# pyprob/pyprob

Hardware: NVIDIA H100
Metric: ic_train_traces_per_sec (higher is better)
Workload: dtype f32

## Files before the change

pyprob_b200/csrc/net.cu:

```cuda
#include <vector>
#include <string.h>
#include <stdlib.h>
#include <stdint.h>

#include "common.cuh"
#include "gemm_simt.cuh"
#include "heads.cuh"
#include "tc_grouped.cuh"
#include "tc_lstm.cuh"
#include "tc_cluster.cuh"
#include "tc_persist.cuh"
#include "obs_mlp.cuh"

using gemm::Problem;

struct HImg {
  float* k_hi = nullptr; float* k_lo = nullptr; float* mn_hi = nullptr; float* mn_lo = nullptr;
  int64_t kb = 0;
};

struct WImg {
  int64_t k_hi = 0, k_lo = 0, mn_hi = 0, mn_lo = 0;
  int kb = 0;
};
// ... 1174 lines not shown
  const int C2 = 2 * (D.type_dim + D.addr_dim);
  const bool one_pass = S <= 4 && H4 <= 2048;
  int max_rows = 0;
  for (int s = 0; s < d.NS; ++s) max_rows = b->step_nrows_host[s] > max_rows ? b->step_nrows_host[s] : max_rows;
  if (one_pass) {
    int slab = (d.R + 2 * PPB_NUM_SMS - 1) / (2 * PPB_NUM_SMS);
    slab = slab < 4 ? 4 : (slab > kRedSlab ? kRedSlab : slab);
    const dim3 g((max_rows + slab - 1) / slab, d.NS);
    const float* wt = d.T > 1 ? w.w_smp_t : w.p_step;
    if (H4 <= 1024)
      k_dgates_reduce<4><<<g, 256, 0, st>>>(dgates, wt, w.smp_emb, b->values, b->step_prev_addr, b->step_row0, b->step_nrows,
                                            b->row_prev, net->d_addrs, H4, S, I, E, w.d_pstep, grad, D.w_ih_off, slab);
    else
      k_dgates_reduce<8><<<g, 256, 0, st>>>(dgates, wt, w.smp_emb, b->values, b->step_prev_addr, b->step_row0, b->step_nrows,
                                            b->row_prev, net->d_addrs, H4, S, I, E, w.d_pstep, grad, D.w_ih_off, slab);
    PPB_LAUNCH_CHECK();
  } else {
    dim3 g((H4 + 31) / 32, d.NS);
    k_step_colsum<<<g, 256, 0, st>>>(dgates, b->step_row0, b->step_nrows, H4, w.d_pstep);
    PPB_LAUNCH_CHECK();
  }
  {
    const int jbs = (C2 + 31) / 32;
    int zsplit = PPB_NUM_SMS / 2 / (jbs * d.NS);
    zsplit = zsplit < 1 ? 1 : (zsplit > 16 ? 16 : zsplit);
    const int nx = jbs * d.NS * zsplit;
    const int nw = (int)(((int64_t)H4 * C2 + H4 + 255) / 256);
    k_pstep_bwd<<<nx + nw, 256, 0, st>>>(w.d_pstep, arena + D.w_ih_off, w.emb_cat, net->d_addrs, net->d_type_off, b->step_addr,
                                         b->step_prev_addr, d.NS, H4, I, E + S, D.type_dim, D.addr_dim, zsplit, nx, grad,
                                         D.w_ih_off, D.b_ih_off, D.b_hh_off);
    PPB_LAUNCH_CHECK();
  }
  if (d.T > 1 && !one_pass) {
    const int slab = 64;
    k_smp_bwd_seg<<<dim3((max_rows + slab - 1) / slab, d.NS), 128, 0, st>>>(dgates, w.w_smp_t, w.smp_emb, b->values,
                                                                           b->step_prev_addr, b->step_row0, b->step_nrows,
                                                                           b->row_prev, net->d_addrs, H4, S, slab, grad);
    PPB_LAUNCH_CHECK();
    int rpb = 1024;
    dim3 g((H4 + 255) / 256, (d.R + rpb - 1) / rpb);
    k_wsmp_grad<<<g, 256, 0, st>>>(dgates, w.smp_emb, d.R, H4, S, I, E, grad + D.w_ih_off, rpb);
    PPB_LAUNCH_CHECK();
  }
  return PPB_OK;
}

}

#include "net_tc.inc"
#include "net_ff.inc"

namespace {

int simt_loss_forward(ppb_net* net, const float* arena, const ppb_batch* b, void* workspace, float* loss_out,
                      int32_t* status_out, float* row_lp_out, int want_grad, cudaStream_t st) {
  PPB_CHECK_ARG(b->row_align == 1, "the SIMT path needs a batch encoded with row_align = 1");
  const ppb_net_desc& D = net->desc;
  Dims d = dims_of(b);
  Ws w = carve(net, d, workspace);
  const int H = D.lstm_dim, H4 = 4 * H, E = D.obs_dim, S = D.sample_dim, I = net->I;

  Builder bl;
  obs_fp32_plan_fwd(bl, D, arena, b->obs, d.B, w, w.obs_emb);
  const int ph_p = (int)bl.phases.size();
  bl.begin();
  bl.add(linear_fwd(w.obs_emb, E, arena + D.w_ih_off, I, nullptr, w.p_obs, H4, d.B, H4, E, 0));
  const int ph_rec0 = (int)bl.phases.size();
  for (int t = 1; t < d.T; ++t) {
    bl.begin();
    int r0 = b->row_off_host[t], n = b->row_off_host[t + 1] - r0, rp = b->row_off_host[t - 1];
    bl.add(linear_fwd(w.h + (int64_t)rp * H, H, arena + D.w_hh_off, H, nullptr, w.gates + (int64_t)r0 * H4, H4, n, H4, H, 0));
  }
  int ph_h1, ph_h2;
  simt_head_fwd(bl, net, arena, b, w, H, ph_h1, ph_h2);
  int rc = upload_and_get(net, bl, w.problems, w.max_problems / 2, st, 0);
  if (rc) return rc;

  PPB_CUDA(cudaMemsetAsync(w.loss_acc, 0, 256, st));
  for (int l = 0; l < ph_p; ++l) { rc = run_phase(bl.phases[l], w.problems, st); if (rc) return rc; }
  rc = launch_step_inputs_fwd(net, arena, b, w, st); if (rc) return rc;
  rc = run_phase(bl.phases[ph_p], w.problems, st, &bl); if (rc) return rc;
  for (int t = 0; t < d.T; ++t) {
    int r0 = b->row_off_host[t], n = b->row_off_host[t + 1] - r0;
    if (t > 0) { rc = run_phase(bl.phases[ph_rec0 + t - 1], w.problems, st, &bl); if (rc) return rc; }
    k_cell_fwd<<<ew_grid((int64_t)n * H), 256, 0, st>>>(w.gates, w.p_obs, w.p_step, w.w_smp_t, w.smp_emb, b->row_step,
                                                       b->row_prev, b->row_trace, w.c, w.h, HImg(), r0, n, H, S, t);
    PPB_LAUNCH_CHECK();
  }
  return simt_head_nll(net, b, w, bl, ph_h1, ph_h2, loss_out, status_out, row_lp_out, want_grad, st);
}

int simt_loss_backward(ppb_net* net, const float* arena, float* grad, const ppb_batch* b, void* workspace, float grad_scale,
                       cudaStream_t st) {
  PPB_CHECK_ARG(b->step_nrows_host, "missing per-step host arrays");
  const ppb_net_desc& D = net->desc;
  Dims d = dims_of(b);
  Ws w = carve(net, d, workspace);
  float* dgates = dgates_ptr(w, workspace);
  const int H = D.lstm_dim, H4 = 4 * H, E = D.obs_dim, I = net->I;

  PPB_CUDA(cudaMemsetAsync(w.d_pstep, 0, (size_t)d.NS * H4 * sizeof(float), st));
  if (grad_scale != 1.0f) {
    k_scale<<<ew_grid((int64_t)d.R * net->out_pad), 256, 0, st>>>(w.d_out, (int64_t)d.R * net->out_pad, grad_scale);
    PPB_LAUNCH_CHECK();
  }

  Builder bl;
  const int ph_dhid = 0, ph_hw = 1;
  simt_head_bwd(bl, net, arena, grad, b, w, H);
  const int ph_rec0 = 2;
  for (int t = d.T - 1; t >= 1; --t) {
    bl.begin();
    int r0 = b->row_off_host[t], n = b->row_off_host[t + 1] - r0;
    bl.add(linear_dx(dgates + (int64_t)r0 * H4, H4, arena + D.w_hh_off, H, w.dh_rec + (int64_t)b->row_off_host[t - 1] * H, H, n, H4, H, 0));
  }
  const int ph_lstm_w = (int)bl.phases.size();
  bl.begin();
  {
    int r1 = b->row_off_host[1 < d.T ? 1 : d.T];
    int n1 = d.R - r1;
    if (n1 > 0) {
      Problem p = linear_dw(dgates + (int64_t)r1 * H4, H4, w.h, H, grad + D.w_hh_off, H, n1, H4, H);
      p.kb_gather = b->row_prev + r1;
      bl.add(p);
    }
    bl.add(linear_dw(w.d_pobs, H4, w.obs_emb, E, grad + D.w_ih_off, I, d.B, H4, E));
    bl.add(linear_dx(w.d_pobs, H4, arena + D.w_ih_off, I, w.d_obs_emb, E, d.B, H4, E, 0));
  }
  const int ph_obs = obs_fp32_plan_bwd(bl, D, arena, grad, b->obs, d.B, w);
  Problem* dprobs = w.problems + w.max_problems / 2;
  int rc = upload_and_get(net, bl, dprobs, w.max_problems / 2, st, 1);
  if (rc) return rc;

  rc = run_phase(bl.phases[ph_dhid], dprobs, st); if (rc) return rc;
  rc = run_phase(bl.phases[ph_hw], dprobs, st); if (rc) return rc;
  rc = launch_head_bias_grad(net, b, w, grad, st); if (rc) return rc;
  for (int t = d.T - 1; t >= 0; --t) {
    int r0 = b->row_off_host[t], n = b->row_off_host[t + 1] - r0;
    int n_next = (t + 1 < d.T) ? b->row_off_host[t + 2] - b->row_off_host[t + 1] : 0;
    if (n_next > 0) { rc = run_phase(bl.phases[ph_rec0 + (d.T - 2 - t)], dprobs, st, &bl); if (rc) return rc; }
    k_cell_bwd<false><<<ew_grid((int64_t)n * H), 256, 0, st>>>(w.gates, w.c, w.dh, w.dh_rec, w.dc, dgates, w.d_pobs, b->row_prev,
                                                       b->row_next, b->row_trace, HImg(), r0, n, H, t, HImg());
    PPB_LAUNCH_CHECK();
  }
  rc = launch_step_inputs_bwd(net, arena, grad, b, w, dgates, st); if (rc) return rc;
  rc = run_phase(bl.phases[ph_lstm_w], dprobs, st, &bl); if (rc) return rc;
  return obs_fp32_bwd(bl, ph_obs, dprobs, D, grad, d.B, w, st);
}

}

extern "C" {

int ppb_net_create(ppb_net** out, const ppb_net_desc* d) {
  PPB_CHECK_ARG(out && d, "null argument");
  PPB_CHECK_ARG(d->network_type == PPB_NET_LSTM || d->network_type == PPB_NET_FEEDFORWARD, "unknown network type");
  if (d->network_type == PPB_NET_FEEDFORWARD)
    PPB_CHECK_ARG(d->obs_dim > 0 && d->lstm_dim == 0 && d->sample_dim == 0 && d->addr_dim == 0 && d->type_dim == 0,
                  "bad dims (a feed-forward net has obs_dim > 0 and no LSTM, sample, address or type embedding)");
  else
    PPB_CHECK_ARG(d->lstm_dim > 0 && d->obs_dim > 0 && d->sample_dim > 0 && d->sample_dim <= 8, "bad dims");
  PPB_CHECK_ARG(d->num_obs > 0 && d->num_obs <= PPB_MAX_OBS, "bad observable count");
  PPB_CHECK_ARG(d->mixture_k > 0 && d->mixture_k <= heads::KMAX, "mixture components must be in [1,32]");
  ppb_net* n = new ppb_net();
  n->desc = *d;
  n->I = d->obs_dim + d->sample_dim + 2 * (d->type_dim + d->addr_dim);
  const char* fc = getenv("PPB_FUSED_CELL");
  n->fused_cell = !(fc && fc[0] == '0');
  const char* hg = getenv("PPB_HOST_STEP_GRAPH");
  n->host_graph = (hg && hg[0] == '0') ? 0 : 1;
  for (int i = 0; i < 16; ++i) PPB_CUDA(cudaEventCreateWithFlags(&n->fork_ev[i], cudaEventDisableTiming));
  for (int i = 0; i < 2; ++i) PPB_CUDA(cudaStreamCreateWithFlags(&n->side[i], cudaStreamNonBlocking));
  *out = n;
  return PPB_OK;
}

int ppb_net_set_tables(ppb_net* net, const ppb_addr_desc* addrs, int32_t n_addrs, const int64_t* type_off,
                       int32_t n_types, int64_t arena_floats) {
  const bool ff = net && net->desc.network_type == PPB_NET_FEEDFORWARD;
  PPB_CHECK_ARG(net && addrs && n_addrs > 0 && (ff ? n_types == 0 : (type_off && n_types > 0)), "bad arguments");
  net->addrs.assign(addrs, addrs + n_addrs);
  net->type_off.assign(type_off, type_off + n_types);
  net->arena_floats = arena_floats;
  int dh = 4, op = 4;
  for (auto& a : net->addrs) {
    PPB_CHECK_ARG(a.family >= 0 && a.family <= PPB_FAMILY_BERNOULLI, "unknown family");
    PPB_CHECK_ARG(a.family != PPB_FAMILY_CATEGORICAL || (a.num_categories > 0 && a.num_categories <= heads::CMAX),
                  "categorical head: 1..128 categories supported");
    PPB_CHECK_ARG(a.family != PPB_FAMILY_BERNOULLI || (a.head_out == 1 && a.smp_in == 1 && a.num_categories == 0),
                  "bernoulli head: head_out = 1, smp_in = 1, num_categories = 0");
    PPB_CHECK_ARG(ff || (a.type_id >= 0 && a.type_id < n_types), "type id out of range");
    if (a.head_hidden > dh) dh = a.head_hidden;
    if (a.head_out > op) op = a.head_out;
  }
  net->dh_pad = (int)align_up(dh, 4);
  net->out_pad = (int)align_up(op, 4);
  if (net->d_addrs) cudaFree(net->d_addrs);
  if (net->d_type_off) cudaFree(net->d_type_off);
  net->d_type_off = nullptr;
  PPB_CUDA(cudaMalloc((void**)&net->d_addrs, sizeof(ppb_addr_desc) * n_addrs));
  PPB_CUDA(cudaMemcpy(net->d_addrs, addrs, sizeof(ppb_addr_desc) * n_addrs, cudaMemcpyHostToDevice));
  if (n_types > 0) {
    PPB_CUDA(cudaMalloc((void**)&net->d_type_off, sizeof(int64_t) * n_types));
    PPB_CUDA(cudaMemcpy(net->d_type_off, type_off, sizeof(int64_t) * n_types, cudaMemcpyHostToDevice));
  }
  return build_weight_images(net);
}

int ppb_net_destroy(ppb_net* net) {
  if (!net) return PPB_OK;
  if (net->d_addrs) cudaFree(net->d_addrs);
  if (net->d_type_off) cudaFree(net->d_type_off);
  for (int i = 0; i < 2; ++i) {
    if (net->h_stage[i]) cudaFreeHost(net->h_stage[i]);
    if (net->ev_stage[i]) cudaEventDestroy(net->ev_stage[i]);
    if (net->h_blob[i]) cudaFreeHost(net->h_blob[i]);
    if (net->ev_blob[i]) cudaEventDestroy(net->ev_blob[i]);
  }
  for (int i = 0; i < 2; ++i) if (net->side[i]) cudaStreamDestroy(net->side[i]);
  for (int i = 0; i < 16; ++i) if (net->fork_ev[i]) cudaEventDestroy(net->fork_ev[i]);
  if (net->wimg) cudaFree(net->wimg);
  if (net->d_pack) cudaFree(net->d_pack);
  if (net->whh_il) cudaFree(net->whh_il);
  if (net->d_lstm_steps) cudaFree(net->d_lstm_steps);
  if (net->host_exec) cudaGraphExecDestroy(net->host_exec);
  if (net->host_stream) cudaStreamDestroy(net->host_stream);
  if (net->host_hyper_dev) cudaFree(net->host_hyper_dev);
  if (net->host_state_dev) cudaFree(net->host_state_dev);
  if (net->host_pin) cudaFreeHost(net->host_pin);
  delete net;
  return PPB_OK;
}

int64_t ppb_ic_workspace_bytes(const ppb_net* net, int32_t n_traces, int32_t n_rows, int32_t t_max, int32_t n_steps,
                               int32_t n_groups) {
  if (!net || n_traces <= 0 || n_rows <= 0) return -1;
  Dims d; d.B = n_traces; d.R = n_rows; d.T = t_max; d.NS = n_steps; d.G = n_groups;
  return simt_region_bytes(net, d) + carve_tc(net, d, nullptr).total_bytes + 1024;
}

int ppb_ic_loss_forward(ppb_net* net, const float* arena, const ppb_batch* b, void* workspace,
                        int64_t workspace_bytes, int precision, float* loss_out, int32_t* status_out,
                        float* row_lp_out, int want_grad, void* stream) {
  int rc = check_batch(net, b);
  if (rc) return rc;
  PPB_CHECK_ARG(arena && workspace, "null arena/workspace");
  PPB_CHECK_ARG(!net->addrs.empty(), "address tables not set");
  PPB_CHECK_ARG(precision >= 0 && precision <= 2, "unknown precision mode");
  Dims d = dims_of(b);
  PPB_CHECK_ARG(workspace_bytes >= ppb_ic_workspace_bytes(net, d.B, d.R, d.T, d.NS, d.G), "workspace too small");
  cudaStream_t st = (cudaStream_t)stream;
  if (net->desc.network_type == PPB_NET_FEEDFORWARD)
    return ff_loss_forward(net, arena, b, workspace, precision, loss_out, status_out, row_lp_out, want_grad, st);
  if (precision != PPB_PREC_FP32_SIMT)
    return tc_loss_forward(net, arena, b, workspace, precision, loss_out, status_out, row_lp_out, want_grad, st);
  return simt_loss_forward(net, arena, b, workspace, loss_out, status_out, row_lp_out, want_grad, st);
}

int ppb_ic_loss_backward(ppb_net* net, const float* arena, float* grad, const ppb_batch* b, void* workspace,
                         int64_t workspace_bytes, int precision, float grad_scale, void* stream) {
  int rc = check_batch(net, b);
  if (rc) return rc;
  PPB_CHECK_ARG(arena && grad && workspace, "null arena/grad/workspace");
  Dims d = dims_of(b);
  PPB_CHECK_ARG(workspace_bytes >= ppb_ic_workspace_bytes(net, d.B, d.R, d.T, d.NS, d.G), "workspace too small");
  cudaStream_t st = (cudaStream_t)stream;
  if (net->desc.network_type == PPB_NET_FEEDFORWARD)
    return ff_loss_backward(net, arena, grad, b, workspace, precision, grad_scale, st);
  if (precision != PPB_PREC_FP32_SIMT) return tc_loss_backward(net, arena, grad, b, workspace, precision, grad_scale, st);
  return simt_loss_backward(net, arena, grad, b, workspace, grad_scale, st);
}

}

namespace {

__global__ void __launch_bounds__(256) k_adam(float* __restrict__ p, const float* __restrict__ g,
                                               float* __restrict__ m, float* __restrict__ v, int64_t n, float lr,
                                               float b1, float b2, float eps, float wd, float bc1, float bc2_sqrt,
                                               float gscale) {
  ppb_pdl_trigger();
  ppb_pdl_wait();
  int64_t n4 = n >> 2;
  float step = lr / bc1;
  for (int64_t q = (int64_t)blockIdx.x * blockDim.x + threadIdx.x; q < n4; q += (int64_t)gridDim.x * blockDim.x) {
    float4 pp = reinterpret_cast<float4*>(p)[q], gg = reinterpret_cast<const float4*>(g)[q];
    float4 mm = reinterpret_cast<float4*>(m)[q], vv = reinterpret_cast<float4*>(v)[q];
    float pa[4] = {pp.x, pp.y, pp.z, pp.w}, ga[4] = {gg.x, gg.y, gg.z, gg.w};
    float ma[4] = {mm.x, mm.y, mm.z, mm.w}, va[4] = {vv.x, vv.y, vv.z, vv.w};
#pragma unroll
    for (int j = 0; j < 4; ++j) ppb_adam_update(pa[j], ga[j], ma[j], va[j], b1, b2, eps, wd, gscale, step, bc2_sqrt);
    reinterpret_cast<float4*>(p)[q] = make_float4(pa[0], pa[1], pa[2], pa[3]);
    reinterpret_cast<float4*>(m)[q] = make_float4(ma[0], ma[1], ma[2], ma[3]);
    reinterpret_cast<float4*>(v)[q] = make_float4(va[0], va[1], va[2], va[3]);
  }
  for (int64_t i = (n4 << 2) + (int64_t)blockIdx.x * blockDim.x + threadIdx.x; i < n;
       i += (int64_t)gridDim.x * blockDim.x) {
    float pi = p[i], mi = m[i], vi = v[i];
    ppb_adam_update(pi, g[i], mi, vi, b1, b2, eps, wd, gscale, step, bc2_sqrt);
    m[i] = mi; v[i] = vi; p[i] = pi;
  }
}

__global__ void __launch_bounds__(256) k_adam_dev(float* __restrict__ p, const float* __restrict__ g,
                                                   float* __restrict__ m, float* __restrict__ v, int64_t n, int vec,
                                                   const float* __restrict__ hyper, long long* __restrict__ step_ctr,
                                                   float* __restrict__ bc1_out, unsigned int* __restrict__ done_ctr) {
  ppb_pdl_trigger();
  ppb_pdl_wait();
  __shared__ float s_bc[2];
  __shared__ long long s_t;
  const int64_t n4 = vec ? (n >> 2) : 0;
  const int64_t stride = (int64_t)gridDim.x * blockDim.x;
  int64_t q = (int64_t)blockIdx.x * blockDim.x + threadIdx.x;
  const float4 z4 = make_float4(0.f, 0.f, 0.f, 0.f);
  float4 gg = z4, mm = z4, vv = z4;
  if (q < n4) {
    gg = reinterpret_cast<const float4*>(g)[q];
    mm = reinterpret_cast<float4*>(m)[q];
    vv = reinterpret_cast<float4*>(v)[q];
  }
  if (threadIdx.x == 0) {
    long long t = *step_ctr + 1;
    s_t = t;
    s_bc[0] = (float)(1.0 - pow((double)hyper[1], (double)t));
    s_bc[1] = (float)sqrt(1.0 - pow((double)hyper[2], (double)t));
  }
  __syncthreads();
  const float lr = hyper[0], b1 = hyper[1], b2 = hyper[2], eps = hyper[3], wd = hyper[4], gscale = hyper[5];
  const float step = lr / s_bc[0], bc2_sqrt = s_bc[1];
  while (q < n4) {
    const bool zero = wd == 0.0f && gg.x == 0.0f && gg.y == 0.0f && gg.z == 0.0f && gg.w == 0.0f && mm.x == 0.0f &&
                      mm.y == 0.0f && mm.z == 0.0f && mm.w == 0.0f && vv.x == 0.0f && vv.y == 0.0f && vv.z == 0.0f &&
                      vv.w == 0.0f;
    if (!zero) {
      float4 pp = reinterpret_cast<float4*>(p)[q];
      ppb_adam_update(pp.x, gg.x, mm.x, vv.x, b1, b2, eps, wd, gscale, step, bc2_sqrt);
      ppb_adam_update(pp.y, gg.y, mm.y, vv.y, b1, b2, eps, wd, gscale, step, bc2_sqrt);
      ppb_adam_update(pp.z, gg.z, mm.z, vv.z, b1, b2, eps, wd, gscale, step, bc2_sqrt);
      ppb_adam_update(pp.w, gg.w, mm.w, vv.w, b1, b2, eps, wd, gscale, step, bc2_sqrt);
      reinterpret_cast<float4*>(p)[q] = pp;
      reinterpret_cast<float4*>(m)[q] = mm;
      reinterpret_cast<float4*>(v)[q] = vv;
    }
    q += stride;
    if (q < n4) {
      gg = reinterpret_cast<const float4*>(g)[q];
      mm = reinterpret_cast<float4*>(m)[q];
      vv = reinterpret_cast<float4*>(v)[q];
    }
  }
  for (int64_t i = (n4 << 2) + (int64_t)blockIdx.x * blockDim.x + threadIdx.x; i < n;
       i += (int64_t)gridDim.x * blockDim.x) {
    float pi = p[i], mi = m[i], vi = v[i];
    ppb_adam_update(pi, g[i], mi, vi, b1, b2, eps, wd, gscale, step, bc2_sqrt);
    m[i] = mi; v[i] = vi; p[i] = pi;
  }
  __syncthreads();
  if (threadIdx.x == 0) {
    __threadfence();
    if (atomicAdd(done_ctr, 1u) == gridDim.x - 1) {
      *step_ctr = s_t;
      *bc1_out = s_bc[0];
      *done_ctr = 0u;
    }
  }
}

__global__ void __launch_bounds__(256) k_cell_infer(const float* __restrict__ rec, const float* __restrict__ p_row,
                                                     const float* __restrict__ w_smp_t,
                                                     const float* __restrict__ smp_emb, float* __restrict__ c,
                                                     float* __restrict__ h, int64_t n, int H, int S, int first) {
  int64_t total = n * H;
  for (int64_t e = (int64_t)blockIdx.x * blockDim.x + threadIdx.x; e < total; e += (int64_t)gridDim.x * blockDim.x) {
    int64_t i = e / H;
    int j = (int)(e % H);
    float pre[4];
#pragma unroll
    for (int g = 0; g < 4; ++g) {
      int col = g * H + j;
      float v = p_row[col];
      if (!first) {
        v += rec[i * 4 * H + col];
        for (int s = 0; s < S; ++s) v = fmaf(smp_emb[i * S + s], w_smp_t[(int64_t)s * 4 * H + col], v);
      }
      pre[g] = v;
    }
    float ig = ppb_cell_sigmoid(pre[0]);
    float fg = ppb_cell_sigmoid(pre[1]);
    float gg = ppb_cell_tanh(pre[2]);
    float og = ppb_cell_sigmoid(pre[3]);
    float cp = first ? 0.0f : c[i * H + j];
    float cn = fg * cp + ig * gg;
    c[i * H + j] = cn;
    h[i * H + j] = og * ppb_cell_tanh(cn);
  }
}

__global__ void k_smp_embed_infer(const float* __restrict__ arena, ppb_addr_desc a, const float* __restrict__ value,
                                  int64_t n, int S, float* __restrict__ smp_emb) {
  for (int64_t e = (int64_t)blockIdx.x * blockDim.x + threadIdx.x; e < n * S; e += (int64_t)gridDim.x * blockDim.x) {
    int64_t i = e / S;
    int j = (int)(e % S);
    smp_emb[e] = fmaxf(smp_embed_pre(arena, a, value[i], j), 0.0f);
  }
}

__global__ void k_step_row_infer(const float* __restrict__ arena, ppb_addr_desc prev, int has_prev, ppb_addr_desc cur,
                                 const int64_t* __restrict__ type_off, int td, int ad, float* __restrict__ row) {
  int C2 = 2 * (td + ad);
  for (int j = threadIdx.x; j < C2; j += blockDim.x) {
    const int64_t o = step_embed_off(type_off, td, ad, j, [&](bool is_prev, const ppb_addr_desc*& a) {
      a = is_prev ? &prev : &cur;
      return !is_prev || has_prev;
    });
    row[j] = o >= 0 ? arena[o] : 0.0f;
  }
}

__global__ void __launch_bounds__(128) k_head_params(const float* __restrict__ out_raw, int out_pad, ppb_addr_desc a,
                                                      int K, const float* __restrict__ prior0, int s0,
                                                      const float* __restrict__ prior1, int s1,
                                                      float* __restrict__ params, int64_t n) {
  for (int64_t i = (int64_t)blockIdx.x * blockDim.x + threadIdx.x; i < n; i += (int64_t)gridDim.x * blockDim.x) {
    const float* x = out_raw + i * out_pad;
    if (a.family == PPB_FAMILY_BERNOULLI) {
      params[i] = heads::bernoulli_prob(x[0]);
    } else if (a.family == PPB_FAMILY_CATEGORICAL) {
      float xs[heads::CMAX], q[heads::CMAX];
      for (int c = 0; c < a.num_categories; ++c) xs[c] = x[c];
      heads::categorical_probs(xs, a.num_categories, q);
      for (int c = 0; c < a.num_categories; ++c) params[i * a.num_categories + c] = q[c];
    } else {
      float xs[3 * heads::KMAX], mean[heads::KMAX], sd[heads::KMAX], pr[heads::KMAX], lo, hi;
      for (int j = 0; j < 3 * K; ++j) xs[j] = x[j];
      float p0 = prior0 ? prior0[i * s0] : 0.0f, p1 = prior1 ? prior1[i * s1] : 0.0f;
      heads::mixture_params(a.family, xs, K, p0, p1, mean, sd, pr, &lo, &hi);
      for (int k = 0; k < K; ++k) {
        params[i * 3 * K + k] = mean[k];
        params[i * 3 * K + K + k] = sd[k];
        params[i * 3 * K + 2 * K + k] = pr[k];
      }
    }
  }
}

struct InferWs {
  HImg h_img, hid_img;
  tcg::Problem* tprobs;
  float *gates, *hid, *out_raw, *smp_emb, *p_row, *emb_row, *w_smp_t;
  float* obs_act[PPB_MAX_OBS][PPB_MAX_FF_LAYERS];
  float* obs_cat;
  float* fin_act[PPB_MAX_FF_LAYERS];
  Problem* problems;
  int64_t max_problems, total_bytes;
};

InferWs carve_infer(const ppb_net* net, int64_t n, void* base) {
  const ppb_net_desc& D = net->desc;
  InferWs w;
  memset(&w, 0, sizeof(w));
  char* p = (char*)base;
  int64_t off = 0;
  auto take = [&](int64_t floats) { float* r = (float*)(p + off); off += align_up(floats * 4, 256); return r; };
  const int H4 = 4 * D.lstm_dim;
  w.gates = take(n * H4);
  w.hid = take(n * net->dh_pad);
  w.out_raw = take(n * net->out_pad);
  w.smp_emb = take(n * D.sample_dim);
  w.p_row = take(H4);
  w.emb_row = take(2 * (D.type_dim + D.addr_dim));
  w.w_smp_t = take((int64_t)D.sample_dim * H4);
  for (int j = 0; j < D.num_obs; ++j)
    for (int l = 0; l + 1 < D.obs_ff[j].num_layers; ++l) w.obs_act[j][l] = take(n * D.obs_ff[j].layers[l].out_dim);
  w.obs_cat = take(n * D.obs_dim);
  for (int l = 0; l + 1 < D.obs_final.num_layers; ++l) w.fin_act[l] = take(n * D.obs_final.layers[l].out_dim);
  w.max_problems = 64 + 2LL * PPB_MAX_OBS * PPB_MAX_FF_LAYERS;
  w.problems = (Problem*)take(w.max_problems * (int64_t)(sizeof(Problem) / 4));
  auto img_k = [&](int64_t rows, int64_t cols) {
    HImg im;
    int64_t nfl = img_floats(rows, cols);
    off = align_up(off, 1024);
    im.kb = (cols + 31) / 32;
    im.k_hi = take(nfl); im.k_lo = take(nfl);
    return im;
  };
  w.h_img = img_k(n, D.lstm_dim);
  w.hid_img = img_k(n, net->dh_pad);
  w.tprobs = (tcg::Problem*)take(8 * (int64_t)(sizeof(tcg::Problem) / 4));
  w.total_bytes = off;
  return w;
}

}

extern "C" {

int ppb_prof_enable(int on) {
  for (auto& sp : g_prof.spans) { cudaEventDestroy(sp.first); cudaEventDestroy(sp.second); }
  g_prof.spans.clear();
  g_prof.flops = 0.0;
  g_prof.launches = 0;
  g_prof.on = on != 0;
  return PPB_OK;
}

int ppb_prof_read(double* total_ms_out, int64_t* launches_out, double* flops_out) {
  double total = 0.0;
  for (auto& sp : g_prof.spans) {
    PPB_CUDA(cudaEventSynchronize(sp.second));
    float ms = 0.0f;
    PPB_CUDA(cudaEventElapsedTime(&ms, sp.first, sp.second));
    total += ms;
  }
  if (total_ms_out) *total_ms_out = total;
  if (launches_out) *launches_out = g_prof.launches;
  if (flops_out) *flops_out = g_prof.flops;
  return PPB_OK;
}

int64_t ppb_sizeof(int which) {
  switch (which) {
    case 0: return sizeof(ppb_net_desc);
    case 1: return sizeof(ppb_addr_desc);
    case 2: return sizeof(ppb_batch);
    case 3: return sizeof(ppb_ff_desc);
    case 4: return sizeof(ppb_linear_desc);
    default: return -1;
  }
}

int ppb_batch_from_image(const void* image_host, const void* image_dev, int64_t image_bytes, ppb_batch* out) {
  PPB_CHECK_ARG(image_host && out, "null image");
  const int64_t* hd = (const int64_t*)image_host;
  PPB_CHECK_ARG(image_bytes >= (int64_t)(PPB_IMAGE_HEADER_WORDS * 8), "image too small");
  PPB_CHECK_ARG(hd[0] == PPB_IMAGE_MAGIC, "bad batch image magic");
  PPB_CHECK_ARG(hd[8] == image_bytes, "image size mismatch");
  memset(out, 0, sizeof(*out));
  out->n_traces = (int32_t)hd[1]; out->n_sub = (int32_t)hd[2]; out->t_max = (int32_t)hd[3];
  out->n_rows = (int32_t)hd[4]; out->n_steps = (int32_t)hd[5]; out->n_groups = (int32_t)hd[6];
  out->obs_in_total = (int32_t)hd[7];
  for (int k = 9; k < 9 + 19; ++k)
    PPB_CHECK_ARG(hd[k] >= PPB_IMAGE_HEADER_WORDS * 8 && hd[k] < image_bytes && (hd[k] & 15) == 0, "bad array offset");
  out->row_align = (int32_t)hd[28];
  PPB_CHECK_ARG(out->row_align == 1 || out->row_align == 128, "row_align must be 1 or 128");
  const char* Hh = (const char*)image_host;
  const char* Dv = (const char*)image_dev;
  out->row_off_host = (const int32_t*)(Hh + hd[9]);
  out->group_addr_host = (const int32_t*)(Hh + hd[10]);
  out->group_start_host = (const int32_t*)(Hh + hd[11]);
  out->step_addr_host = (const int32_t*)(Hh + hd[13]);
  out->step_row0_host = (const int32_t*)(Hh + hd[15]);
  out->step_nrows_host = (const int32_t*)(Hh + hd[16]);
  out->step_t_host = (const int32_t*)(Hh + hd[26]);
  out->step_prev_row0_host = (const int32_t*)(Hh + hd[27]);
  if (Dv) {
    out->trace_sub = (const int32_t*)(Dv + hd[12]);
    out->step_addr = (const int32_t*)(Dv + hd[13]);
    out->step_prev_addr = (const int32_t*)(Dv + hd[14]);
    out->step_row0 = (const int32_t*)(Dv + hd[15]);
    out->step_nrows = (const int32_t*)(Dv + hd[16]);
    out->row_step = (const int32_t*)(Dv + hd[17]);
    out->row_prev = (const int32_t*)(Dv + hd[18]);
    out->values = (const float*)(Dv + hd[19]);
    out->prior0 = (const float*)(Dv + hd[20]);
    out->prior1 = (const float*)(Dv + hd[21]);
    out->obs = (const float*)(Dv + hd[22]);
    out->head_rows = (const int32_t*)(Dv + hd[23]);
    out->row_trace = (const int32_t*)(Dv + hd[24]);
    out->row_next = (const int32_t*)(Dv + hd[25]);
    out->step_t = (const int32_t*)(Dv + hd[26]);
    out->step_prev_row0 = (const int32_t*)(Dv + hd[27]);
    out->group_addr = (const int32_t*)(Dv + hd[10]);
    out->group_start = (const int32_t*)(Dv + hd[11]);
  }
  return PPB_OK;
}

int ppb_adam_step(float* arena, const float* grad, float* exp_avg, float* exp_avg_sq, int64_t n, float lr, float beta1,
                  float beta2, float eps, float weight_decay, int64_t step, float grad_scale, void* stream) {
  PPB_CHECK_ARG(arena && grad && exp_avg && exp_avg_sq && n > 0 && step >= 1, "bad arguments");
  double bc1 = 1.0 - pow((double)beta1, (double)step), bc2 = 1.0 - pow((double)beta2, (double)step);
  PPB_CUDA(ppb_launch(k_adam, dim3(ppb_grid_for(n, 256, 4)), dim3(256), 0, (cudaStream_t)stream, 0, 0, arena, grad, exp_avg,
                      exp_avg_sq, n, lr, beta1, beta2, eps, weight_decay, (float)bc1, (float)sqrt(bc2), grad_scale));
  PPB_LAUNCH_CHECK();
  return PPB_OK;
}

int ppb_adam_step_dev(float* arena, const float* grad, float* exp_avg, float* exp_avg_sq, int64_t n,
                      const float* hyper_dev, void* state_dev, void* stream) {
  PPB_CHECK_ARG(arena && grad && exp_avg && exp_avg_sq && hyper_dev && state_dev && n > 0, "bad arguments");
  const int vec = ((((uintptr_t)arena | (uintptr_t)grad | (uintptr_t)exp_avg | (uintptr_t)exp_avg_sq) & 15) == 0) ? 1 : 0;
  PPB_CUDA(ppb_launch(k_adam_dev, dim3(ppb_grid_for(n, 256, 4)), dim3(256), 0, (cudaStream_t)stream, 0, 0, arena, grad,
                      exp_avg, exp_avg_sq, n, vec, hyper_dev, (long long*)state_dev, (float*)((char*)state_dev + 8),
                      (unsigned int*)((char*)state_dev + 12)));
  PPB_LAUNCH_CHECK();
  return PPB_OK;
}

int ppb_net_refresh_weights(ppb_net* net, const float* arena, void* stream) {
  PPB_CHECK_ARG(net && arena && net->wimg, "bad arguments (tables not set?)");
  k_pack_table<<<dim3(net->pack_tiles, 8), 256, 0, (cudaStream_t)stream>>>(arena, net->d_pack, (int)net->pack.size(), net->wimg);
  PPB_LAUNCH_CHECK();
  return PPB_OK;
}

int64_t ppb_ic_infer_workspace_bytes(const ppb_net* net, int64_t n) {
  if (!net || n <= 0) return -1;
  return carve_infer(net, n, nullptr).total_bytes + 1024;
}

int ppb_ic_embed_observe(ppb_net* net, const float* arena, const float* obs, float* obs_emb_out, int64_t n,
                         void* workspace, int64_t workspace_bytes, void* stream) {
  PPB_CHECK_ARG(net && arena && obs && obs_emb_out && workspace && n > 0, "bad arguments");
  PPB_CHECK_ARG(workspace_bytes >= ppb_ic_infer_workspace_bytes(net, n), "workspace too small");
  cudaStream_t st = (cudaStream_t)stream;
  InferWs w = carve_infer(net, n, workspace);
  if (net->wimg) {
    int rcw = ppb_net_refresh_weights(net, arena, stream);
    if (rcw) return rcw;
  }
  Builder bl;
  obs_fp32_plan_fwd(bl, net->desc, arena, obs, (int)n, w, obs_emb_out);
  int rc = upload_and_get(net, bl, w.problems, w.max_problems, st, 5);
  if (rc) return rc;
  for (auto& ph : bl.phases) { rc = run_phase(ph, w.problems, st); if (rc) return rc; }
  return PPB_OK;
}

int ppb_ic_infer_step(ppb_net* net, const float* arena, const float* obs_emb, int obs_emb_row_stride, int32_t prev_addr,
                      const float* prev_value, int32_t cur_addr, const float* prior0, int prior0_stride,
                      const float* prior1, int prior1_stride, float* h, float* c, float* params_out, int64_t n,
                      void* workspace, int64_t workspace_bytes, int precision, void* stream) {
  const bool ff = net && net->desc.network_type == PPB_NET_FEEDFORWARD;
  PPB_CHECK_ARG(net && arena && obs_emb && (ff || (h && c)) && params_out && workspace && n > 0, "bad arguments");
  PPB_CHECK_ARG(cur_addr >= 0 && cur_addr < (int)net->addrs.size(), "unknown current address");
  PPB_CHECK_ARG(workspace_bytes >= ppb_ic_infer_workspace_bytes(net, n), "workspace too small");
  if (ff) {
    if (obs_emb_row_stride != 0) {
      ppb_set_error("ppb_ic_infer_step: per-particle observation embeddings are not supported yet (stride must be 0)");
      return PPB_ENOTSUP;
    }
    const ppb_net_desc& D = net->desc;
    cudaStream_t st = (cudaStream_t)stream;
    InferWs w = carve_infer(net, n, workspace);
    const ppb_addr_desc cur = net->addrs[cur_addr];
    const int E = D.obs_dim;
    Builder bl;
    bl.begin();
    bl.add(linear_fwd(obs_emb, E, arena + cur.w1_off, E, arena + cur.b1_off, w.hid, net->dh_pad, 1, cur.head_hidden, E, gemm::kRelu));
    bl.begin();
    bl.add(linear_fwd(w.hid, net->dh_pad, arena + cur.w2_off, cur.head_hidden, arena + cur.b2_off, w.out_raw, net->out_pad, 1,
                      cur.head_out, cur.head_hidden, 0));
    int rc = upload_and_get(net, bl, w.problems, w.max_problems, st, 5);
    if (rc) return rc;
    rc = run_phase(bl.phases[0], w.problems, st); if (rc) return rc;
    rc = run_phase(bl.phases[1], w.problems, st); if (rc) return rc;
    k_head_params<<<ew_grid(n, 128), 128, 0, st>>>(w.out_raw, 0, cur, D.mixture_k, prior0, prior0_stride, prior1, prior1_stride,
                                                   params_out, n);
    PPB_LAUNCH_CHECK();
    return PPB_OK;
  }
  PPB_CHECK_ARG(prev_addr < (int)net->addrs.size(), "unknown previous address");
  PPB_CHECK_ARG(prev_addr < 0 || prev_value, "previous value missing");
  if (obs_emb_row_stride != 0) {
    ppb_set_error("ppb_ic_infer_step: per-particle observation embeddings are not supported yet (stride must be 0)");
    return PPB_ENOTSUP;
  }
  (void)precision;
  const ppb_net_desc& D = net->desc;
  cudaStream_t st = (cudaStream_t)stream;
  InferWs w = carve_infer(net, n, workspace);
  const int H = D.lstm_dim, H4 = 4 * H, E = D.obs_dim, S = D.sample_dim, I = net->I, C2 = 2 * (D.type_dim + D.addr_dim);
  const ppb_addr_desc cur = net->addrs[cur_addr];
  const bool first = prev_addr < 0;
  const ppb_addr_desc prev = first ? cur : net->addrs[prev_addr];

  Builder bl;
  bl.begin();
  bl.add(linear_fwd(w.emb_row, C2, arena + D.w_ih_off + E + S, I, arena + D.b_ih_off, w.p_row, H4, 1, H4, C2, 0));
  bl.begin();
  bl.add(linear_fwd(obs_emb, E, arena + D.w_ih_off, I, arena + D.b_hh_off, w.p_row, H4, 1, H4, E, gemm::kAccumulate));
  bl.begin();
  if (!first) bl.add(linear_fwd(h, H, arena + D.w_hh_off, H, nullptr, w.gates, H4, (int)n, H4, H, 0));
  bl.begin();
  bl.add(linear_fwd(h, H, arena + cur.w1_off, H, arena + cur.b1_off, w.hid, net->dh_pad, (int)n, cur.head_hidden, H, gemm::kRelu));
  bl.begin();
  bl.add(linear_fwd(w.hid, net->dh_pad, arena + cur.w2_off, cur.head_hidden, arena + cur.b2_off, w.out_raw, net->out_pad,
                    (int)n, cur.head_out, cur.head_hidden, 0));
  int rc = upload_and_get(net, bl, w.problems, w.max_problems, st, 5);
  if (rc) return rc;
  const bool use_tc = precision != PPB_PREC_FP32_SIMT && (H % 32 == 0) && net->wimg != nullptr;
  TcBuilder tb;
  if (use_tc) {
    tb.begin();
    if (!first) {
      tcg::Problem p = TP0();
      p.a = op_k(w.h_img.k_hi, w.h_img.k_lo, (int)w.h_img.kb, 0, 0);
      p.b = wk(net, net->w_hh);
      p.M = (int)n; p.N = H4; p.K = H; p.c = w.gates; p.ldc = H4;
      tb.add(p);
    }
    tb.begin();
    {
      tcg::Problem p = TP0();
      p.a = op_k(w.h_img.k_hi, w.h_img.k_lo, (int)w.h_img.kb, 0, 0);
      p.b = wk(net, net->w1[cur_addr]);
      p.M = (int)n; p.N = cur.head_hidden; p.K = H;
      p.flags = tcg::kRelu; p.bias = arena + cur.b1_off;
      p.o_k_hi = w.hid_img.k_hi; p.o_k_lo = w.hid_img.k_lo; p.o_kb = (int)w.hid_img.kb;
      tb.add(p);
    }
    tb.begin();
    {
      tcg::Problem p = TP0();
      p.a = op_k(w.hid_img.k_hi, w.hid_img.k_lo, (int)w.hid_img.kb, 0, 0);
      p.b = wk(net, net->w2[cur_addr]);
      p.M = (int)n; p.N = cur.head_out; p.K = cur.head_hidden;
      p.bias = arena + cur.b2_off; p.c = w.out_raw; p.ldc = net->out_pad;
      tb.add(p);
    }
    rc = upload_cached(net, 6, tb.probs.data(), tb.probs.size() * sizeof(tcg::Problem), w.tprobs, st);
    if (rc) return rc;
  }
  const dim3 pack_grid((unsigned)((n + 127) / 128), 4);
  k_step_row_infer<<<1, 128, 0, st>>>(arena, prev, first ? 0 : 1, cur, net->d_type_off, D.type_dim, D.addr_dim, w.emb_row);
  PPB_LAUNCH_CHECK();
  rc = run_phase(bl.phases[0], w.problems, st); if (rc) return rc;
  rc = run_phase(bl.phases[1], w.problems, st); if (rc) return rc;
  if (!first) {
    k_wsmp_transpose<<<ew_grid(S * H4), 256, 0, st>>>(arena + D.w_ih_off, I, E, S, H4, w.w_smp_t);
    PPB_LAUNCH_CHECK();
    k_smp_embed_infer<<<ew_grid(n * S), 256, 0, st>>>(arena, prev, prev_value, n, S, w.smp_emb);
    PPB_LAUNCH_CHECK();
    if (use_tc) {
      k_pack_rows<<<pack_grid, 256, 0, st>>>(h, (int)n, H, H, w.h_img);
      PPB_LAUNCH_CHECK();
      rc = run_tc_phase(tb.phases[0], w.tprobs, precision, st, 0); if (rc) return rc;
    } else {
      rc = run_phase(bl.phases[2], w.problems, st); if (rc) return rc;
    }
  }
  k_cell_infer<<<ew_grid(n * H), 256, 0, st>>>(w.gates, w.p_row, w.w_smp_t, w.smp_emb, c, h, n, H, S, first ? 1 : 0);
  PPB_LAUNCH_CHECK();
  if (use_tc) {
    k_pack_rows<<<pack_grid, 256, 0, st>>>(h, (int)n, H, H, w.h_img);
    PPB_LAUNCH_CHECK();
    rc = run_tc_phase(tb.phases[1], w.tprobs, precision, st, 2); if (rc) return rc;
    rc = run_tc_phase(tb.phases[2], w.tprobs, precision, st, 0); if (rc) return rc;
  } else {
    rc = run_phase(bl.phases[3], w.problems, st); if (rc) return rc;
    rc = run_phase(bl.phases[4], w.problems, st); if (rc) return rc;
  }
  k_head_params<<<ew_grid(n, 128), 128, 0, st>>>(w.out_raw, net->out_pad, cur, D.mixture_k, prior0, prior0_stride, prior1,
                                                 prior1_stride, params_out, n);
  PPB_LAUNCH_CHECK();
  return PPB_OK;
}

int ppb_ic_train_step_host(ppb_net* net, float* arena, float* grad_arena, float* exp_avg, float* exp_avg_sq,
                           int64_t arena_floats, const void* batch_image_host, int64_t batch_image_bytes,
                           void* batch_image_dev, void* workspace, int64_t workspace_bytes, int precision, float lr,
                           float beta1, float beta2, float eps, float weight_decay, int64_t step, float* loss_host,
                           int32_t* status_host, void* stream) {
  PPB_CHECK_ARG(net && arena && grad_arena && exp_avg && exp_avg_sq && batch_image_host && batch_image_dev && workspace,
                "null argument");
  cudaStream_t st = (cudaStream_t)stream;
  ppb_batch b;
  int rc = ppb_batch_from_image(batch_image_host, batch_image_dev, batch_image_bytes, &b);
  if (rc) return rc;
  Dims d = dims_of(&b);
  int64_t need = ppb_ic_workspace_bytes(net, d.B, d.R, d.T, d.NS, d.G);
  PPB_CHECK_ARG(workspace_bytes >= need + 256, "workspace too small (need ppb_ic_workspace_bytes + 256)");
  float* loss_dev = (float*)((char*)workspace + need);
  int32_t* status_dev = (int32_t*)(loss_dev + 1);

  if (!net->host_graph || g_prof.on) {
    PPB_CUDA(cudaMemcpyAsync(batch_image_dev, batch_image_host, batch_image_bytes, cudaMemcpyHostToDevice, st));
    PPB_CUDA(cudaMemsetAsync(grad_arena, 0, arena_floats * sizeof(float), st));
    rc = ppb_ic_loss_forward(net, arena, &b, workspace, need, precision, loss_dev, status_dev, nullptr, 1, stream);
    if (rc) return rc;
    rc = ppb_ic_loss_backward(net, arena, grad_arena, &b, workspace, need, precision, 1.0f, stream);
    if (rc) return rc;
    rc = ppb_adam_step(arena, grad_arena, exp_avg, exp_avg_sq, arena_floats, lr, beta1, beta2, eps, weight_decay, step, 1.0f,
                       stream);
    if (rc) return rc;
    if (loss_host) PPB_CUDA(cudaMemcpyAsync(loss_host, loss_dev, sizeof(float), cudaMemcpyDeviceToHost, st));
    if (status_host) PPB_CUDA(cudaMemcpyAsync(status_host, status_dev, sizeof(int32_t), cudaMemcpyDeviceToHost, st));
    PPB_CUDA(cudaStreamSynchronize(st));
    return PPB_OK;
  }

  if (!net->host_stream) {
    PPB_CUDA(cudaStreamCreateWithFlags(&net->host_stream, cudaStreamNonBlocking));
    PPB_CUDA(cudaMalloc((void**)&net->host_hyper_dev, 6 * sizeof(float)));
    PPB_CUDA(cudaMalloc(&net->host_state_dev, 16));
    PPB_CUDA(cudaMemset(net->host_state_dev, 0, 16));
    net->host_step_dev = 0;
  }
  cudaStream_t hs = net->host_stream;
  if (net->host_pin_cap < batch_image_bytes + 16) {
    PPB_CUDA(cudaStreamSynchronize(hs));
    if (net->host_pin) cudaFreeHost(net->host_pin);
    net->host_pin_cap = 2 * batch_image_bytes + 16;
    PPB_CUDA(cudaHostAlloc((void**)&net->host_pin, (size_t)net->host_pin_cap, cudaHostAllocDefault));
  }
  char* const pin_img = net->host_pin;
  char* const pin_res = net->host_pin + (net->host_pin_cap - 16);
  uint64_t key = fnv1a(&d, sizeof(d));
  key = fnv1a(&batch_image_bytes, sizeof(batch_image_bytes), key);
  key = fnv1a(&pin_img, sizeof(pin_img), key);
  key = fnv1a(b.row_off_host, sizeof(int32_t) * (d.T + 1), key);
  key = fnv1a(b.group_addr_host, sizeof(int32_t) * d.G, key);
  key = fnv1a(b.group_start_host, sizeof(int32_t) * (d.G + 1), key);
  key = fnv1a(b.step_addr_host, sizeof(int32_t) * d.NS, key);
  key = fnv1a(b.step_row0_host, sizeof(int32_t) * d.NS, key);
  key = fnv1a(b.step_nrows_host, sizeof(int32_t) * d.NS, key);
  key = fnv1a(b.step_t_host, sizeof(int32_t) * d.NS, key);
  key = fnv1a(b.step_prev_row0_host, sizeof(int32_t) * d.NS, key);
  const void* ptrs[8] = {arena, grad_arena, exp_avg, exp_avg_sq, batch_image_dev, workspace, (const void*)(intptr_t)precision,
                         (const void*)(intptr_t)arena_floats};
  key = fnv1a(ptrs, sizeof(ptrs), key);
  key = fnv1a(&net->arena_floats, sizeof(net->arena_floats), key);
  if (key != net->host_key) {
    if (net->host_exec) { cudaGraphExecDestroy(net->host_exec); net->host_exec = nullptr; }
    net->host_key = key;
    net->host_seen = 0;
  }
  rc = stream_after(net, st, hs);
  if (rc) return rc;
  memcpy(pin_img, batch_image_host, (size_t)batch_image_bytes);
  const float hyper[6] = {lr, beta1, beta2, eps, weight_decay, 1.0f};
  if (memcmp(hyper, net->host_hyper, sizeof(hyper)) != 0) {
    memcpy(net->host_hyper, hyper, sizeof(hyper));
    PPB_CUDA(cudaMemcpyAsync(net->host_hyper_dev, net->host_hyper, sizeof(hyper), cudaMemcpyHostToDevice, hs));
  }
  if (net->host_step_dev != step - 1) {
    const int64_t prev = step - 1;
    PPB_CUDA(cudaMemcpyAsync(net->host_state_dev, &prev, sizeof(prev), cudaMemcpyHostToDevice, hs));
    PPB_CUDA(cudaStreamSynchronize(hs));
  }
  auto enqueue = [&](cudaStream_t q) -> int {
    PPB_CUDA(cudaMemcpyAsync(batch_image_dev, pin_img, batch_image_bytes, cudaMemcpyHostToDevice, q));
    PPB_CUDA(cudaMemsetAsync(grad_arena, 0, arena_floats * sizeof(float), q));
    int r = ppb_ic_loss_forward(net, arena, &b, workspace, need, precision, loss_dev, status_dev, nullptr, 1, (void*)q);
    if (r) return r;
    r = ppb_ic_loss_backward(net, arena, grad_arena, &b, workspace, need, precision, 1.0f, (void*)q);
    if (r) return r;
    r = ppb_adam_step_dev(arena, grad_arena, exp_avg, exp_avg_sq, arena_floats, net->host_hyper_dev, net->host_state_dev,
                          (void*)q);
    if (r) return r;
    PPB_CUDA(cudaMemcpyAsync(pin_res, loss_dev, 8, cudaMemcpyDeviceToHost, q));
    return PPB_OK;
  };
  if (net->host_exec) {
    PPB_CUDA(cudaGraphLaunch(net->host_exec, hs));
  } else if (net->host_seen >= 1) {
    cudaGraph_t graph = nullptr;
    PPB_CUDA(cudaStreamBeginCapture(hs, cudaStreamCaptureModeThreadLocal));
    rc = enqueue(hs);
    cudaError_t ce = cudaStreamEndCapture(hs, &graph);
    if (rc || ce != cudaSuccess || !graph) {
      if (graph) cudaGraphDestroy(graph);
      cudaGetLastError();
      if (rc) return rc;
      ppb_set_error("ppb_ic_train_step_host: graph capture failed: %s", cudaGetErrorString(ce));
      return (int)ce;
    }
    ce = cudaGraphInstantiate(&net->host_exec, graph, 0);
    cudaGraphDestroy(graph);
    if (ce != cudaSuccess) {
      net->host_exec = nullptr;
      ppb_set_error("ppb_ic_train_step_host: cudaGraphInstantiate: %s", cudaGetErrorString(ce));
      return (int)ce;
    }
    PPB_CUDA(cudaGraphLaunch(net->host_exec, hs));
  } else {
    rc = enqueue(hs);
    if (rc) return rc;
  }
  net->host_seen += 1;
  net->host_step_dev = step;
  PPB_CUDA(cudaStreamSynchronize(hs));
  if (loss_host) memcpy(loss_host, pin_res, sizeof(float));
  if (status_host) memcpy(status_host, pin_res + sizeof(float), sizeof(int32_t));
  return PPB_OK;
}

}
```

Measured before the change: 1.586 million.

## Restructure device Adam kernel to overlap state loads with PDL wait

The device-side Adam kernel now loads optimizer state (m, v, and p when state is nonzero) before waiting on the preceding kernel via PDL, so only the gradient read depends on the producer. It processes three float4 vectors per thread per chunk, prefetches the next chunk into L2, uses cache-global loads, and moves the PDL trigger to the end of the kernel with a fence. The launch enables the PDL attribute and sizes the grid for five blocks per SM. The aim is to hide memory latency and launch gaps between backward and optimizer. The trade-offs are added register pressure and reliance on PDL ordering for correctness.

```diff
diff --git a/pyprob_b200/csrc/net.cu b/pyprob_b200/csrc/net.cu
--- a/pyprob_b200/csrc/net.cu
+++ b/pyprob_b200/csrc/net.cu
@@ -1500,58 +1500,83 @@
   }
 }
 
-__global__ void __launch_bounds__(256) k_adam_dev(float* __restrict__ p, const float* __restrict__ g,
-                                                   float* __restrict__ m, float* __restrict__ v, int64_t n, int vec,
-                                                   const float* __restrict__ hyper, long long* __restrict__ step_ctr,
-                                                   float* __restrict__ bc1_out, unsigned int* __restrict__ done_ctr) {
-  ppb_pdl_trigger();
-  ppb_pdl_wait();
+constexpr int kAdamThreads = 256, kAdamVec = 3, kAdamBlocksPerSm = 5;
+
+__device__ __forceinline__ bool ppb_is_zero4(float4 a) { return a.x == 0.0f && a.y == 0.0f && a.z == 0.0f && a.w == 0.0f; }
+
+__global__ void __launch_bounds__(kAdamThreads, kAdamBlocksPerSm)
+    k_adam_dev(float* __restrict__ p, const float* __restrict__ g, float* __restrict__ m, float* __restrict__ v, int64_t n,
+               int vec, const float* __restrict__ hyper, long long* __restrict__ step_ctr, float* __restrict__ bc1_out,
+               unsigned int* __restrict__ done_ctr) {
   __shared__ float s_bc[2];
   __shared__ long long s_t;
-  const int64_t n4 = vec ? (n >> 2) : 0;
-  const int64_t stride = (int64_t)gridDim.x * blockDim.x;
-  int64_t q = (int64_t)blockIdx.x * blockDim.x + threadIdx.x;
-  const float4 z4 = make_float4(0.f, 0.f, 0.f, 0.f);
-  float4 gg = z4, mm = z4, vv = z4;
-  if (q < n4) {
-    gg = reinterpret_cast<const float4*>(g)[q];
-    mm = reinterpret_cast<float4*>(m)[q];
-    vv = reinterpret_cast<float4*>(v)[q];
-  }
+  const float lr = hyper[0], b1 = hyper[1], b2 = hyper[2], eps = hyper[3], wd = hyper[4], gscale = hyper[5];
   if (threadIdx.x == 0) {
     long long t = *step_ctr + 1;
     s_t = t;
-    s_bc[0] = (float)(1.0 - pow((double)hyper[1], (double)t));
-    s_bc[1] = (float)sqrt(1.0 - pow((double)hyper[2], (double)t));
+    s_bc[0] = (float)(1.0 - pow((double)b1, (double)t));
+    s_bc[1] = (float)sqrt(1.0 - pow((double)b2, (double)t));
+  }
+  const int64_t n4 = vec ? (n >> 2) : 0;
+  const int64_t chunk = (int64_t)kAdamThreads * kAdamVec;
+  const int64_t chunk_stride = (int64_t)gridDim.x * chunk;
+  float4* const p4 = reinterpret_cast<float4*>(p);
+  float4* const m4 = reinterpret_cast<float4*>(m);
+  float4* const v4 = reinterpret_cast<float4*>(v);
+  const float4 z4 = make_float4(0.f, 0.f, 0.f, 0.f);
+  float4 mm[kAdamVec], vv[kAdamVec], pp[kAdamVec];
+  auto stateless = [&](int j) { return wd == 0.0f && ppb_is_zero4(mm[j]) && ppb_is_zero4(vv[j]); };
+  auto load_state = [&](int64_t c0) {
+#pragma unroll
+    for (int j = 0; j < kAdamVec; ++j) {
+      const int64_t q = c0 + j * kAdamThreads;
+      mm[j] = z4; vv[j] = z4; pp[j] = z4;
+      if (q < n4) { mm[j] = __ldcg(m4 + q); vv[j] = __ldcg(v4 + q); }
+    }
+#pragma unroll
+    for (int j = 0; j < kAdamVec; ++j) {
+      const int64_t q = c0 + j * kAdamThreads;
+      if (q < n4 && !stateless(j)) pp[j] = __ldcg(p4 + q);
+    }
+  };
+  const int64_t c_first = (int64_t)blockIdx.x * chunk + threadIdx.x;
+  load_state(c_first);
+#pragma unroll
+  for (int j = 0; j < kAdamVec; ++j) {
+    const int64_t q = c_first + chunk_stride + j * kAdamThreads;
+    if (q < n4) {
+      asm volatile("prefetch.global.L2 [%0];" ::"l"(m4 + q));
+      asm volatile("prefetch.global.L2 [%0];" ::"l"(v4 + q));
+      asm volatile("prefetch.global.L2 [%0];" ::"l"(p4 + q));
+    }
   }
   __syncthreads();
-  const float lr = hyper[0], b1 = hyper[1], b2 = hyper[2], eps = hyper[3], wd = hyper[4], gscale = hyper[5];
   const float step = lr / s_bc[0], bc2_sqrt = s_bc[1];
-  while (q < n4) {
-    const bool zero = wd == 0.0f && gg.x == 0.0f && gg.y == 0.0f && gg.z == 0.0f && gg.w == 0.0f && mm.x == 0.0f &&
-                      mm.y == 0.0f && mm.z == 0.0f && mm.w == 0.0f && vv.x == 0.0f && vv.y == 0.0f && vv.z == 0.0f &&
-                      vv.w == 0.0f;
-    if (!zero) {
-      float4 pp = reinterpret_cast<float4*>(p)[q];
-      ppb_adam_update(pp.x, gg.x, mm.x, vv.x, b1, b2, eps, wd, gscale, step, bc2_sqrt);
-      ppb_adam_update(pp.y, gg.y, mm.y, vv.y, b1, b2, eps, wd, gscale, step, bc2_sqrt);
-      ppb_adam_update(pp.z, gg.z, mm.z, vv.z, b1, b2, eps, wd, gscale, step, bc2_sqrt);
-      ppb_adam_update(pp.w, gg.w, mm.w, vv.w, b1, b2, eps, wd, gscale, step, bc2_sqrt);
-      reinterpret_cast<float4*>(p)[q] = pp;
-      reinterpret_cast<float4*>(m)[q] = mm;
-      reinterpret_cast<float4*>(v)[q] = vv;
-    }
-    q += stride;
-    if (q < n4) {
-      gg = reinterpret_cast<const float4*>(g)[q];
-      mm = reinterpret_cast<float4*>(m)[q];
-      vv = reinterpret_cast<float4*>(v)[q];
+  ppb_pdl_wait();
+  for (int64_t c0 = c_first; c0 < n4; c0 += chunk_stride) {
+    if (c0 != c_first) load_state(c0);
+#pragma unroll
+    for (int j = 0; j < kAdamVec; ++j) {
+      const int64_t q = c0 + j * kAdamThreads;
+      if (q >= n4) continue;
+      const float4 gg = __ldcg(reinterpret_cast<const float4*>(g) + q);
+      if (stateless(j)) {
+        if (ppb_is_zero4(gg)) continue;
+        pp[j] = p4[q];
+      }
+      ppb_adam_update(pp[j].x, gg.x, mm[j].x, vv[j].x, b1, b2, eps, wd, gscale, step, bc2_sqrt);
+      ppb_adam_update(pp[j].y, gg.y, mm[j].y, vv[j].y, b1, b2, eps, wd, gscale, step, bc2_sqrt);
+      ppb_adam_update(pp[j].z, gg.z, mm[j].z, vv[j].z, b1, b2, eps, wd, gscale, step, bc2_sqrt);
+      ppb_adam_update(pp[j].w, gg.w, mm[j].w, vv[j].w, b1, b2, eps, wd, gscale, step, bc2_sqrt);
+      p4[q] = pp[j];
+      m4[q] = mm[j];
+      v4[q] = vv[j];
     }
   }
   for (int64_t i = (n4 << 2) + (int64_t)blockIdx.x * blockDim.x + threadIdx.x; i < n;
        i += (int64_t)gridDim.x * blockDim.x) {
     float pi = p[i], mi = m[i], vi = v[i];
-    ppb_adam_update(pi, g[i], mi, vi, b1, b2, eps, wd, gscale, step, bc2_sqrt);
+    ppb_adam_update(pi, __ldcg(g + i), mi, vi, b1, b2, eps, wd, gscale, step, bc2_sqrt);
     m[i] = mi; v[i] = vi; p[i] = pi;
   }
   __syncthreads();
@@ -1563,6 +1588,8 @@
       *done_ctr = 0u;
     }
   }
+  __threadfence();
+  ppb_pdl_trigger();
 }
 
 __global__ void __launch_bounds__(256) k_cell_infer(const float* __restrict__ rec, const float* __restrict__ p_row,
@@ -1789,9 +1816,9 @@
                       const float* hyper_dev, void* state_dev, void* stream) {
   PPB_CHECK_ARG(arena && grad && exp_avg && exp_avg_sq && hyper_dev && state_dev && n > 0, "bad arguments");
   const int vec = ((((uintptr_t)arena | (uintptr_t)grad | (uintptr_t)exp_avg | (uintptr_t)exp_avg_sq) & 15) == 0) ? 1 : 0;
-  PPB_CUDA(ppb_launch(k_adam_dev, dim3(ppb_grid_for(n, 256, 4)), dim3(256), 0, (cudaStream_t)stream, 0, 0, arena, grad,
-                      exp_avg, exp_avg_sq, n, vec, hyper_dev, (long long*)state_dev, (float*)((char*)state_dev + 8),
-                      (unsigned int*)((char*)state_dev + 12)));
+  PPB_CUDA(ppb_launch(k_adam_dev, dim3(ppb_grid_for(n, kAdamThreads, 4 * kAdamVec, kAdamBlocksPerSm)), dim3(kAdamThreads), 0,
+                      (cudaStream_t)stream, 1, 0, arena, grad, exp_avg, exp_avg_sq, n, vec, hyper_dev, (long long*)state_dev,
+                      (float*)((char*)state_dev + 8), (unsigned int*)((char*)state_dev + 12)));
   PPB_LAUNCH_CHECK();
   return PPB_OK;
 }
```

Result: faster. 1.624 million, median of 6 (+2.4%).
